# HandBrake/HandBrake

Hardware: AMD Instinct MI355X
Metric: filtered frames/sec, 1080p YUV420p NLMeans+decomb chain (higher is better)
Workload: dtype u8 (f32 NLMeans weights, 16-bit fixed-point scaler as zimg, sharpen mix = the reference's f64 expression, as one f32 multiply where init proves that equal); 1 GPU; BASELINE configs[3]: decomb(31, EEDI2 bob) -> nlmeans medium -> cropscale lanczos 1920x1080 -> 3840x2160 -> lapsharp, 1080i YUV420P 8-bit in, inputs resident in HBM; input=1920x1080, output=3840x2160, streams_per_gpu=1, content=interlaced, stream_frames=48, stage_streams=2, parallelism=1 GPU(s) x 1 independent stream(s), device=AMD Radeon Graphics (gfx950:sramecc+:xnack-, 256 CUs)

## Files before the change

handbrake_amd/csrc/eedi2.hip:

```cpp
#include "eedi2_common.h"
#include "eedi2_vote.h"
#include "eedi2_dirmap_vote.h"
#include "eedi2_dense.h"
#include "eedi2_engine.h"
#include "eedi2_mask_cells.h"
#include "eedi2_corner.h"

#include <atomic>
#include <algorithm>

namespace {

constexpr int PEAK = 255, NEUTRAL = 128;
constexpr int EEDI_MAX_FIELDS = EEDI_MAX_BATCH;
constexpr size_t GUARD = 32768;

__constant__ uint8_t c_limlut[33] = { 6, 6, 7, 7, 8, 8, 9, 9, 9, 10, 10, 11, 11, 12, 12, 12, 12, 12, 12, 12,
                                      12, 12, 12, 12, 12, 12, 12, 12, 12, 12, 12, 255, 255 };

constexpr int LIM_N = 33, LIM_PAD = 40;
__device__ __forceinline__ void lim_fill(uint8_t *tab, int tid)
{
    if (tid < LIM_N) tab[tid] = c_limlut[tid];
}
// ... 708 lines not shown
        {
            if (k == 1 && tid >= 64) break;
            const int i = tid + k * CD_W;
    #pragma unroll
            for (int m = 0; m < NM; m++)
            {
                const uint64_t w = __ballot(s_band[NS + m][i] == PEAK);
                if (lane == 0) s_bits[m][i >> 6] = w;
            }
        }
        __syncthreads();
    }
#ifdef HBHIP_DEV_STATS
    if (tid == 0) { CD_STAT(0, 1); CD_STAT(1, count != 0); CD_STAT(2, count); CD_STAT(7, dense); }
#endif
    if (R >= 4 && dense)
    {
        constexpr int RD = R >= 4 ? R : 1;
        const int lx = tid, px = x0 + lx, b = lx + CD_HALO - 1;
        const int startu = max(-px + 1, -maxdt), stopu = min(width - 2 - px, maxdt);
        uint64_t range = 0;
        if (stopu >= startu)
        {
            const int nb = stopu - startu + 1;
            range = (nb >= 64 ? ~0ull : ((1ull << nb) - 1ull)) << (startu + maxdt);
        }
        uint64_t win[RD + 2];
#pragma unroll
        for (int m = 0; m < RD + 2; m++) win[m] = calc_dir_window(s_bits[m], b - maxdt, lenmask);
        uint32_t up[RD], dn[RD], act = 0, inactive = 0;
#pragma unroll
        for (int j = 0; j < RD; j++)
        {
            const uint8_t *mr = &s_band[NS + j + 1][CD_HALO + lx];
            const bool a = px >= 1 && px < width - 1 && mr[0] == PEAK && (mr[-1] == PEAK || mr[1] == PEAK);
            const uint64_t pass = a ? range & win[j] & (__brevll(win[j + 2]) >> (64 - len)) : 0ull;
            const uint64_t npass = ~pass;
            up[j] = (uint32_t)(npass >> maxdt);
            dn[j] = __brev((uint32_t)npass << (31 - maxdt));
            act |= (uint32_t)a << j;
            inactive |= (up[j] | dn[j]) & ((2u << maxdt) - 1u);
        }
        if (__any(act != 0))
        {
            const uint32_t *tr = &s_tri[0][b];
            if (__all(inactive == 0))
                calc_dir_dense_vote<RD, false, RD, 0>(tr, maxdt, up, dn, act, nt13, nt19, &s_out[0][lx]);
            else
            {
                constexpr int RH = RD >= 8 ? RD / 2 : RD;
                calc_dir_dense_vote<RH, true, RD, 0>(tr, maxdt, up, dn, act, nt13, nt19, &s_out[0][lx]);
                if constexpr (RH < RD) calc_dir_dense_vote<RD - RH, true, RD, RH>(tr, maxdt, up, dn, act, nt13, nt19, &s_out[0][lx]);
            }
#ifdef HBHIP_DEV_STATS
            if (lane == 0) { CD_STAT(8, 1); CD_STAT(9, __all(inactive == 0)); }
#endif
        }
        __syncthreads();
    }
    else if (count)
    {
        for (int p = tid; p < count; p += CD_W)
        {
            const uint32_t id = s_list[p];
            const int j = (int)(id >> 8), lx = (int)(id & 255u), y = y0 + j, px = x0 + lx, b = lx + CD_HALO - 1;
            const int startu = max(-px + 1, -maxdt), stopu = min(width - 2 - px, maxdt);
            uint64_t pass = 0;
            if (stopu >= startu)
            {
                const int nb = stopu - startu + 1;
                pass = (nb >= 64 ? ~0ull : ((1ull << nb) - 1ull)) << (startu + maxdt);
                if (y != 1)          pass &= calc_dir_window(s_bits[j], b - maxdt, lenmask);
                if (y != height - 2) pass &= __brevll(calc_dir_window(s_bits[j + 2], b - maxdt, lenmask)) >> (64 - len);
            }
#ifdef HBHIP_DEV_STATS
            {
                int n = __popcll(pass), mx = n, sm = n, ln = 1;
                for (int o = 32; o; o >>= 1) { mx = max(mx, __shfl_xor(mx, o)); sm += __shfl_xor(sm, o); ln += __shfl_xor(ln, o); }
                const uint64_t act = __ballot(1);
                if (lane == __ffsll((unsigned long long)act) - 1) { CD_STAT(3, 1); CD_STAT(4, sm); CD_STAT(5, mx); CD_STAT(6, ln); }
            }
#endif
            const uint32_t *tr = &s_tri[j][b];
            int out;
            if (len <= 32)
                out = edge ? calc_dir_search<true, uint32_t>(tr, (uint32_t)pass, maxdt, y == 1, y == height - 2, nt13, nt19)
                           : calc_dir_search<false, uint32_t>(tr, (uint32_t)pass, maxdt, false, false, nt13, nt19);
            else
                out = edge ? calc_dir_search<true, uint64_t>(tr, pass, maxdt, y == 1, y == height - 2, nt13, nt19)
                           : calc_dir_search<false, uint64_t>(tr, pass, maxdt, false, false, nt13, nt19);
            s_out[j][lx] = (uint8_t)out;
        }
        __syncthreads();
    }
#pragma unroll
    for (int jr = 0; jr < R; jr += CD_W / 64)
    {
        const int j = jr + (tid >> 6), y = y0 + j, xb = x0 + 4 * lane;
        if (j < R && y < height && xb < pitch)
            *reinterpret_cast<uint32_t *>(Q.c + (size_t)y * pitch + xb) = pad_bytes(reinterpret_cast<const uint32_t *>(&s_out[j][0])[lane], xb, width, padv);
    }
}


__device__ __forceinline__ int dir_map_px(int u0, int u1, int u2, int c0, int c1, int c2, int n0, int n1, int n2,
                                          bool up_ok, bool dn_ok, int expand, const uint8_t *limlut)
{
    const bool h0 = up_ok && u0 != PEAK, h1 = up_ok && u1 != PEAK, h2 = up_ok && u2 != PEAK;
    const bool h3 = c0 != PEAK, h4 = !expand && c1 != PEAK, h5 = c2 != PEAK;
    const bool h6 = dn_ok && n0 != PEAK, h7 = dn_ok && n1 != PEAK, h8 = dn_ok && n2 != PEAK;
    const int u = h0 + h1 + h2 + h3 + h4 + h5 + h6 + h7 + h8;
    if (u < (expand ? 5 : 4)) return expand ? c1 : PEAK;
    int v0 = h0 ? u0 : ABSENT, v1 = h1 ? u1 : ABSENT, v2 = h2 ? u2 : ABSENT;
    int v3 = h3 ? c0 : ABSENT, v4 = h4 ? c1 : ABSENT, v5 = h5 ? c2 : ABSENT;
    int v6 = h6 ? n0 : ABSENT, v7 = h7 ? n1 : ABSENT, v8 = h8 ? n2 : ABSENT;
    int s0 = v0, s1 = v1, s2 = v2, s3 = v3, s4 = v4, s5 = v5, s6 = v6, s7 = v7, s8 = v8;
    const int mid = mid9(s0, s1, s2, s3, s4, s5, s6, s7, s8, u);
    const int lim = limlut[iabs(mid - NEUTRAL) >> 2];
    int sum = 0, count = 0;
    vote1(v0, mid, lim, sum, count); vote1(v1, mid, lim, sum, count); vote1(v2, mid, lim, sum, count);
    vote1(v3, mid, lim, sum, count); vote1(v4, mid, lim, sum, count); vote1(v5, mid, lim, sum, count);
    vote1(v6, mid, lim, sum, count); vote1(v7, mid, lim, sum, count); vote1(v8, mid, lim, sum, count);
    const int val = dmv_vote_avg(sum + mid, count + 1);
    if (expand) return count >= 5 ? (val & 0xff) : c1;
    if (count < 4 || (count < 5 && c1 == PEAK)) return PEAK;
    return val & 0xff;
}

__device__ __forceinline__ uint32_t ff_bytes(uint32_t v)
{
    return (((v & 0x7f7f7f7fu) + 0x01010101u) & v) & 0x80808080u;
}

constexpr uint32_t PK_ABSENT_HI = 0x7f00u;
__device__ __forceinline__ u16x2 limlut2(u16x2 i)
{
    const u16x2 g = pk_lt(pk1(7), i);
    const u16x2 l = __builtin_elementwise_min((u16x2)(((i - g) >> 1) + pk1(6)), pk1(12));
    const u16x2 big = pk_lt(pk1(30), i) * pk1(255);
    return __builtin_elementwise_max(l, big);
}
#define PK_BYTES(hi, lo, a, b) __builtin_amdgcn_perm((hi), (lo), 0x0c000c00u | ((uint32_t)(b) << 16) | (uint32_t)(a))

template <int PAIRS>
__device__ __forceinline__ uint32_t dir_map_quad(const Win12 &wu, const Win12 &wc, const Win12 &wd)
{
    return ::dir_map_quad<PAIRS>(wu.w0, wu.w1, wu.w2, wc.w0, wc.w1, wc.w2, wd.w0, wd.w1, wd.w2);
}

__global__ __launch_bounds__(256) void k_dir_map4(P3 P)
{
    FIELD_PLANE(P);
    const int x = 4 * (blockIdx.x * blockDim.x + threadIdx.x);
    const int y = blockIdx.y * blockDim.y + threadIdx.y;
    const int pitch = P.pitch[pl], width = P.width[pl], height = P.height[pl];
    if (x >= width || y >= height) return;
    uint8_t *o = Q.c + (size_t)y * pitch + x;
    if (maskless)
    {
        const int out[4] = { PEAK, PEAK, PEAK, PEAK };
        st4(o, out, x, width);
        return;
    }
    const uint8_t *dc = Q.b + (size_t)y * pitch + x;
    const uint32_t own = *reinterpret_cast<const uint32_t *>(dc);
    uint32_t res = own;
    if (y >= 1 && y < height - 1)
    {
        const uint32_t m0 = *reinterpret_cast<const uint32_t *>(Q.a + (size_t)y * pitch + x);
        const uint32_t work = (ff_bytes(m0) >> 7) & bytes_in(x, 1, width - 1);
        if (work)
        {
            asm volatile("" ::: "memory");
            const Win12 wc = ldwin(dc), wu = ldwin(dc - (ptrdiff_t)pitch), wd = ldwin(dc + (ptrdiff_t)pitch);
            const uint32_t votes = dir_map_quad<3>(wu, wc, wd);
            const uint32_t sel = (work << 8) - work;
            res = (res & ~sel) | (votes & sel);
        }
    }
    int out[4] = { (int)(res & 0xff), (int)((res >> 8) & 0xff), (int)((res >> 16) & 0xff), (int)(res >> 24) };
    st4(o, out, x, width);
}

__device__ __forceinline__ uint32_t live3(const Win12 &w, uint32_t &centre)
{
    const uint32_t n0 = (~ff_bytes(w.w0) >> 7) & 0x01010101u, n1 = (~ff_bytes(w.w1) >> 7) & 0x01010101u, n2 = (~ff_bytes(w.w2) >> 7) & 0x01010101u;
    centre = n1;
    return __builtin_amdgcn_alignbyte(n1, n0, 3) + n1 + __builtin_amdgcn_alignbyte(n2, n1, 1);
}

#ifndef DC_THREAD_ROWS
#define DC_THREAD_ROWS 4
#endif
constexpr int DC_R = DC_THREAD_ROWS, DC_ROWS = 4 * DC_R;
__global__ __launch_bounds__(256) void k_dir_map_c(P3 P)
{
    __shared__ __attribute__((aligned(16))) uint8_t s_out[DC_ROWS][256];
    __shared__ uint16_t s_list[DC_ROWS * 256];
    __shared__ int s_count;
    __shared__ uint8_t s_lim[LIM_PAD];
    FIELD_PLANE(P);
    const int rb = blockIdx.y * DC_ROWS;
    const int bx0 = 4 * (blockIdx.x * 64), x = bx0 + 4 * threadIdx.x;
    const int pitch = P.pitch[pl], width = P.width[pl], height = P.height[pl];
    if (bx0 >= width || rb >= height) return;
    if (maskless)
    {
        if (x < width)
        {
            const int out[4] = { PEAK, PEAK, PEAK, PEAK };
#pragma unroll
            for (int h = 0; h < DC_R; h++)
            {
                const int y = rb + (int)threadIdx.y + 4 * h;
                if (y < height) st4(Q.c + (size_t)y * pitch + x, out, x, width);
            }
        }
        return;
    }
    const int tid = threadIdx.y * 64 + threadIdx.x;
    if (tid == 0) s_count = 0;
    lim_fill(s_lim, tid);
    __syncthreads();
    uint32_t own[DC_R], m0[DC_R], cand[DC_R];
#pragma unroll
    for (int h = 0; h < DC_R; h++)
    {
        const int y = rb + (int)threadIdx.y + 4 * h;
        own[h] = 0; m0[h] = 0;
        if (x < width && y < height)
        {
            own[h] = *reinterpret_cast<const uint32_t *>(Q.b + (size_t)y * pitch + x);
            if (y >= 1 && y < height - 1)
                m0[h] = *reinterpret_cast<const uint32_t *>(Q.a + (size_t)y * pitch + x);
        }
    }
    Win12 wc[DC_R], wu[DC_R], wd[DC_R];
#pragma unroll
    for (int h = 0; h < DC_R; h++)
    {
        const int y = rb + (int)threadIdx.y + 4 * h;
        cand[h] = (ff_bytes(m0[h]) >> 7) & bytes_in(x, 1, width - 1) & (ff_bytes(own[h]) >> 7);
        wc[h] = wu[h] = wd[h] = Win12{ 0u, 0u, 0u };
        if (cand[h])
        {
            const uint8_t *dc = Q.b + (size_t)y * pitch + x;
            wc[h] = ldwin(dc); wu[h] = ldwin(dc - (ptrdiff_t)pitch); wd[h] = ldwin(dc + (ptrdiff_t)pitch);
        }
    }
#pragma unroll
    for (int h = 0; h < DC_R; h++)
    {
        const int lr = (int)threadIdx.y + 4 * h, y = rb + lr;
        if (x < width && y < height)
        {
            if (cand[h])
            {
                uint32_t nc, nu, nd;
                const uint32_t s3c = live3(wc[h], nc), s3u = live3(wu[h], nu), s3d = live3(wd[h], nd);
                const uint32_t u = s3c - nc + s3u + s3d;
                const uint32_t enough = ((u + (uint32_t)(0x80 - 5) * 0x01010101u) >> 7) & 0x01010101u;
                const uint32_t sortpx = cand[h] & enough;
                if (sortpx)
                {
                    int at = atomicAdd(&s_count, __popc(sortpx));
#pragma unroll
                    for (int k = 0; k < 4; k++)
                        if ((sortpx >> (8 * k)) & 1u) s_list[at++] = (uint16_t)((lr << 8) | (4 * threadIdx.x + k));
                }
                (void)nu; (void)nd;
            }
            *reinterpret_cast<uint32_t *>(&s_out[lr][4 * threadIdx.x]) = own[h];
        }
    }
    __syncthreads();
    const int count = s_count;
    for (int i = tid; i < count; i += 256)
    {
        const int e = s_list[i], ly = e >> 8, lx = e & 255;
        const uint8_t *c = Q.b + (size_t)(rb + ly) * pitch + bx0 + lx;
        const uint8_t *up = c - (ptrdiff_t)pitch, *dn = c + (ptrdiff_t)pitch;
        s_out[ly][lx] = (uint8_t)dir_map_px(up[-1], up[0], up[1], c[-1], c[0], c[1], dn[-1], dn[0], dn[1], true, true, 1, s_lim);
    }
    __syncthreads();
#pragma unroll
    for (int h = 0; h < DC_R; h++)
    {
        const int lr = (int)threadIdx.y + 4 * h, y = rb + lr;
        if (x < width && y < height)
        {
            const uint32_t v = *reinterpret_cast<const uint32_t *>(&s_out[lr][4 * threadIdx.x]);
            uint8_t *o = Q.c + (size_t)y * pitch + x;
            if (x + 3 < width) *reinterpret_cast<uint32_t *>(o) = v;
            else for (int k = 0; k < 4 && x + k < width; k++) o[k] = (uint8_t)(v >> (8 * k));
        }
    }
}

#ifndef FE_ROWS
#define FE_ROWS 14
#endif
constexpr int FE_R = FE_ROWS, FE_LW = 68;

__device__ __forceinline__ void fe_expand_row(const uint32_t (*s_f)[FE_LW], int lr, int tx, uint32_t cand, bool up_ok, bool dn_ok,
                                              uint8_t (*s_out)[256], uint16_t *s_list, int *s_count)
{
    const uint32_t own = s_f[lr + 1][tx + 1];
    cand &= ff_bytes(own) >> 7;
    if (cand)
    {
        const Win12 none = { 0xffffffffu, 0xffffffffu, 0xffffffffu };
        const Win12 wc = { s_f[lr + 1][tx], own, s_f[lr + 1][tx + 2] };
        const Win12 wu = up_ok ? Win12{ s_f[lr][tx], s_f[lr][tx + 1], s_f[lr][tx + 2] } : none;
        const Win12 wd = dn_ok ? Win12{ s_f[lr + 2][tx], s_f[lr + 2][tx + 1], s_f[lr + 2][tx + 2] } : none;
        uint32_t nc, nu, nd;
        const uint32_t s3c = live3(wc, nc), s3u = live3(wu, nu), s3d = live3(wd, nd);
        const uint32_t u = s3c - nc + s3u + s3d;
        const uint32_t enough = ((u + (uint32_t)(0x80 - 5) * 0x01010101u) >> 7) & 0x01010101u;
        const uint32_t sortpx = cand & enough;
        if (sortpx)
        {
            int at = atomicAdd(s_count, __popc(sortpx));
#pragma unroll
            for (int k = 0; k < 4; k++)
                if ((sortpx >> (8 * k)) & 1u) s_list[at++] = (uint16_t)((lr << 8) | (4 * tx + k));
        }
        (void)nu; (void)nd;
    }
    *reinterpret_cast<uint32_t *>(&s_out[lr][4 * tx]) = own;
}

template <int STEP, bool POST>
__global__ __launch_bounds__(256) void k_dir_map_fe(P3 P, uint32_t padv)
{
    __shared__ uint32_t s_f[FE_R + 2][FE_LW];
    __shared__ __attribute__((aligned(16))) uint8_t s_out[FE_R][256];
    __shared__ uint16_t s_list[FE_R * 256];
    __shared__ int s_count;
    __shared__ uint8_t s_lim[LIM_PAD];
    FIELD_PLANE(P);
    const int y0 = STEP == 1 ? 1 : 2 - tff, par = STEP == 1 ? 0 : (y0 & 1);
    const int rb = blockIdx.y * FE_R;
    const int bx0 = 256 * blockIdx.x, x = bx0 + 4 * threadIdx.x;
    const int pitch = P.pitch[pl], width = P.width[pl], height = P.height[pl];
    if (bx0 >= pitch || STEP * rb >= height) return;
    auto row_ok = [&](int y) { return STEP == 1 ? (y >= 1 && y < height - 1) : (y >= y0 && y < height - 1); };
    if (maskless)
    {
        if (x < pitch)
            for (int lr = threadIdx.y; lr < FE_R; lr += 4)
#pragma unroll
                for (int i = 0; i < STEP; i++)
                    if (STEP * (rb + lr) + i < height)
                    {
                        const size_t at = (size_t)(STEP * (rb + lr) + i) * pitch + x;
                        *reinterpret_cast<uint32_t *>(Q.c + at) = pad_bytes(0xffffffffu, x, width, padv);
                        if (POST && x < width) { const int out[4] = { PEAK, PEAK, PEAK, PEAK }; st4(Q.d + at, out, x, width); }
                    }
        return;
    }
    const int tid = threadIdx.y * 64 + threadIdx.x;
    if (tid == 0) s_count = 0;
    lim_fill(s_lim, tid);
    constexpr int NCOPY = STEP == 1 ? 1 : (FE_R + 3) / 4;
    uint32_t vcopy[NCOPY];
    if (STEP != 1)
#pragma unroll
        for (int h = 0; h < NCOPY; h++)
        {
            const int lr = threadIdx.y + 4 * h, yc = 2 * (rb + lr) + 1 - par;
            vcopy[h] = (lr < FE_R && yc < height && x < width) ? *reinterpret_cast<const uint32_t *>(Q.b + (size_t)yc * pitch + x) : 0u;
        }
    auto filtered = [&](int r, int xx, auto side) -> uint32_t {
        constexpr int SIDE = decltype(side)::value;
        const int y = STEP * r + par;
        if (r < 0 || y >= height || xx < 0 || xx >= width) return 0u;
        const uint8_t *dc = Q.b + (size_t)y * pitch + xx;
        const uint32_t own = *reinterpret_cast<const uint32_t *>(dc);
        if (!row_ok(y)) return own;
        const uint8_t *mk = Q.a + (size_t)y * pitch + xx;
        const uint32_t m0 = *reinterpret_cast<const uint32_t *>(STEP == 1 ? mk : mk - (ptrdiff_t)pitch);
        const uint32_t m1 = STEP == 1 ? 0u : *reinterpret_cast<const uint32_t *>(mk + pitch);
        uint32_t work = ((ff_bytes(m0) | ff_bytes(m1)) >> 7) & bytes_in(xx, 1, width - 1);
        if (SIDE < 0) work &= 0xff000000u;
        if (SIDE > 0) work &= 0x000000ffu;
        uint32_t res = own;
        if (work)
        {
            asm volatile("" ::: "memory");
            const bool up_ok = STEP == 1 || y > 1, dn_ok = STEP == 1 || y < height - 2;
            const Win12 none = { 0xffffffffu, 0xffffffffu, 0xffffffffu };
            const Win12 wc = ldwin(dc), wu = up_ok ? ldwin(dc - (ptrdiff_t)STEP * pitch) : none, wd = dn_ok ? ldwin(dc + (ptrdiff_t)STEP * pitch) : none;
            const uint32_t votes = dir_map_quad<(SIDE < 0 ? 2 : SIDE > 0 ? 1 : 3)>(wu, wc, wd);
            const uint32_t sel = (work << 8) - work;
            res = (res & ~sel) | (votes & sel);
        }
        return res;
    };
    for (int lr = threadIdx.y; lr < FE_R + 2; lr += 4) s_f[lr][threadIdx.x + 1] = filtered(rb - 1 + lr, x, std::integral_constant<int, 0>());
    static_assert(FE_R + 2 <= 64, "a lane per ring row");
    if (threadIdx.y == 0 && (int)threadIdx.x < FE_R + 2) s_f[threadIdx.x][0] = filtered(rb - 1 + (int)threadIdx.x, bx0 - 4, std::integral_constant<int, -1>());
    if (threadIdx.y == 1 && (int)threadIdx.x < FE_R + 2) s_f[threadIdx.x][65] = filtered(rb - 1 + (int)threadIdx.x, bx0 + 256, std::integral_constant<int, 1>());
    __syncthreads();
    for (int lr = threadIdx.y; lr < FE_R; lr += 4)
    {
        const int y = STEP * (rb + lr) + par;
        if (x >= width || y >= height) continue;
        uint32_t cand = 0;
        if (row_ok(y))
        {
            const uint8_t *mk = Q.a + (size_t)y * pitch + x;
            const uint32_t m0 = *reinterpret_cast<const uint32_t *>(STEP == 1 ? mk : mk - (ptrdiff_t)pitch);
            const uint32_t m1 = STEP == 1 ? 0u : *reinterpret_cast<const uint32_t *>(mk + pitch);
            cand = ((ff_bytes(m0) | ff_bytes(m1)) >> 7) & bytes_in(x, 1, width - 1);
        }
        fe_expand_row(s_f, lr, threadIdx.x, cand, STEP == 1 || y > 1, STEP == 1 || y < height - 2, s_out, s_list, &s_count);
    }
    __syncthreads();
    const int count = s_count;
    for (int i = tid; i < count; i += 256)
    {
        const int e = s_list[i], ly = e >> 8, lx = e & 255;
        const int y = STEP * (rb + ly) + par;
        const uint8_t *c = reinterpret_cast<const uint8_t *>(&s_f[ly + 1][1]) + lx;
        const uint8_t *up = c - 4 * FE_LW, *dn = c + 4 * FE_LW;
        s_out[ly][lx] = (uint8_t)dir_map_px(up[-1], up[0], up[1], c[-1], c[0], c[1], dn[-1], dn[0], dn[1],
                                            STEP == 1 || y > 1, STEP == 1 || y < height - 2, 1, s_lim);
    }
    __syncthreads();
#pragma unroll
    for (int h = 0; h < (FE_R + 3) / 4; h++)
    {
        const int lr = threadIdx.y + 4 * h, y = STEP * (rb + lr) + par;
        if (lr >= FE_R || x >= pitch) continue;
        auto put_d = [&](int yy, uint32_t v) {
            if (x >= width) return;
            uint8_t *o = Q.d + (size_t)yy * pitch + x;
            if (x + 3 < width) *reinterpret_cast<uint32_t *>(o) = v;
            else for (int k = 0; k < 4 && x + k < width; k++) o[k] = (uint8_t)(v >> (8 * k));
        };
        if (y < height)
        {
            const uint32_t v = x < width ? *reinterpret_cast<const uint32_t *>(&s_out[lr][4 * threadIdx.x]) : 0u;
            *reinterpret_cast<uint32_t *>(Q.c + (size_t)y * pitch + x) = pad_bytes(v, x, width, padv);
            if (POST) put_d(y, s_f[lr + 1][threadIdx.x + 1]);
            if (POST && x < width && row_ok(y))
            {
                const size_t at = (size_t)y * pitch + x;
                const uint32_t om4 = *reinterpret_cast<const uint32_t *>(Q.b + at);
                uint8_t *d = Q.f + at;
                const uint32_t up4 = *reinterpret_cast<const uint32_t *>(d - pitch), dn4 = *reinterpret_cast<const uint32_t *>(d + pitch);
                const uint32_t cur4 = *reinterpret_cast<const uint32_t *>(d);
                int out[4];
                bool any = false;
#pragma unroll
                for (int k = 0; k < 4; k++)
                {
                    const int nm = (v >> (8 * k)) & 0xffu, om = (om4 >> (8 * k)) & 0xffu;
                    const int lim = s_lim[iabs(nm - NEUTRAL) >> 2];
                    const bool fix = iabs(nm - om) > lim && om != PEAK && om != NEUTRAL;
                    out[k] = fix ? (int)((((up4 >> (8 * k)) & 0xffu) + ((dn4 >> (8 * k)) & 0xffu) + 1) >> 1) : (int)((cur4 >> (8 * k)) & 0xffu);
                    any |= fix;
                }
                if (any) st4(d, out, x, width);
            }
        }
        if (STEP != 1)
        {
            const int yc = 2 * (rb + lr) + 1 - par;
            if (yc < height)
            {
                *reinterpret_cast<uint32_t *>(Q.c + (size_t)yc * pitch + x) = pad_bytes(vcopy[h < NCOPY ? h : 0], x, width, padv);
                if (POST) put_d(yc, vcopy[h < NCOPY ? h : 0]);
            }
        }
    }
}


constexpr int FM_W = 256, FM_R = 4, FM_HALO = 8, FM_LW = FM_W + 2 * FM_HALO;

__device__ __forceinline__ int fm_step(uint32_t s, uint32_t c, uint32_t ref, int lim)
{
    const int off_s = lim - (int)__builtin_amdgcn_sad_u16(s, ref, 0u), off_c = lim - (int)__builtin_amdgcn_sad_u16(c, ref, 0u);
    return (off_s & (int)(s - 255u)) | (off_c & (int)(c - 255u)) | (509 - (int)c - (int)s);
}

__global__ __launch_bounds__(256) void k_filter_map(P3 P)
{
    __shared__ __attribute__((aligned(16))) uint8_t s_d[FM_R + 2][FM_LW];
    FIELD_PLANE(P);
    const int pitch = P.pitch[pl], width = P.width[pl], height = P.height[pl];
    const int bx0 = blockIdx.x * FM_W, by0 = blockIdx.y * FM_R;
    if (bx0 >= width || by0 >= height) return;
    const int tid = threadIdx.y * 64 + threadIdx.x;
    const int x = bx0 + 4 * threadIdx.x, y = by0 + threadIdx.y;
    if (maskless)
    {
        if (x < width && y < height)
        {
            uint8_t *o = Q.c + (size_t)y * pitch + x;
            if (x + 3 < width) *reinterpret_cast<uint32_t *>(o) = 0xffffffffu;
            else for (int k = 0; k < 4 && x + k < width; k++) o[k] = (uint8_t)PEAK;
        }
        return;
    }
    const bool inside = x < width && y < height;
    uint32_t m4 = 0, own = 0;
    if (inside)
    {
        own = *reinterpret_cast<const uint32_t *>(Q.b + (size_t)y * pitch + x);
        if (y >= 1 && y < height - 1) m4 = *reinterpret_cast<const uint32_t *>(Q.a + (size_t)y * pitch + x);
    }
    uint32_t cand = ((ff_bytes(m4) & ~ff_bytes(own)) >> 7) & bytes_in(x, 1, width - 1);
    if (!__syncthreads_or(cand != 0u))
    {
        if (inside)
        {
            uint8_t *o = Q.c + (size_t)y * pitch + x;
            if (x + 3 < width) *reinterpret_cast<uint32_t *>(o) = own;
            else for (int k = 0; k < 4 && x + k < width; k++) o[k] = (uint8_t)(own >> (8 * k));
        }
        return;
    }
    {
        static_assert((FM_R + 2) * (FM_LW / 4) <= 2 * 256, "two staged dwords per thread");
        uint32_t v[2] = { 0u, 0u };
#pragma unroll
        for (int k = 0; k < 2; k++)
        {
            const int i = tid + 256 * k, r = i / (FM_LW / 4), c4 = i - r * (FM_LW / 4);
            const int yy = by0 - 1 + r, col = bx0 - FM_HALO + 4 * c4;
            if (i < (FM_R + 2) * (FM_LW / 4) && yy >= 0 && yy < height && col >= 0 && col < pitch)
                v[k] = *reinterpret_cast<const uint32_t *>(Q.b + (size_t)yy * pitch + col);
        }
#pragma unroll
        for (int k = 0; k < 2; k++)
            if (tid + 256 * k < (FM_R + 2) * (FM_LW / 4)) reinterpret_cast<uint32_t *>(&s_d[0][0])[tid + 256 * k] = v[k];
    }
    __syncthreads();
    if (!inside) return;
    const uint8_t *rc = &s_d[threadIdx.y + 1][FM_HALO + 4 * threadIdx.x];
    uint32_t out4 = own;
#pragma unroll 1
    for (int k = 0; k < 4; k++)
    {
        if (!((cand >> (8 * k)) & 1u)) continue;
        const int xx = x + k;
        const uint8_t *dc = rc + k, *dp = dc - FM_LW, *dn = dc + FM_LW;
        const uint32_t ref = dc[0];
        int dir = ((int)ref - NEUTRAL) >> 2;
        const int lim = max(iabs(dir) * 2, 12 << 2);
        dir >>= 2;
        const int neg = min(dir, 0), pos = max(dir, 0);
        const int tf = max(-xx, neg), tt = min(width - xx - 1, pos), bf = max(-xx, -pos), bt = min(width - xx - 1, -neg);
        const int n = max(tt - tf, bt - bf);
        int any_t = 0, any_b = 0;
        for (int i = 0; i <= n; i++)
        {
            const int jt = min(tf + i, tt), jb = min(bf + i, bt);
            any_t |= fm_step(dp[jt], dc[jt], ref, lim);
            any_b |= fm_step(dn[jb], dc[jb], ref, lim);
        }
        if ((any_t & any_b) < 0) out4 |= 0xffu << (8 * k);
    }
    uint8_t *o = Q.c + (size_t)y * pitch + x;
    if (x + 3 < width) *reinterpret_cast<uint32_t *>(o) = out4;
    else for (int k = 0; k < 4 && x + k < width; k++) o[k] = (uint8_t)(out4 >> (8 * k));
}

template <int K>
__device__ __forceinline__ uint32_t mark_pair(const Win12 &wa, const Win12 &wb)
{
    u16x2 v[6];
    {
        const Win12 *rows[2] = { &wa, &wb };
#pragma unroll
        for (int r = 0; r < 2; r++)
        {
            const uint32_t w0 = rows[r]->w0, w1 = rows[r]->w1, w2 = rows[r]->w2;
            if (K == 0)
            {
                v[3 * r + 0] = pk(PK_BYTES(w1, w0, 3, 4));
                v[3 * r + 1] = pk(PK_BYTES(w1, w0, 4, 5));
                v[3 * r + 2] = pk(PK_BYTES(w1, w0, 5, 6));
            }
            else
            {
                v[3 * r + 0] = pk(PK_BYTES(w1, w0, 5, 6));
                v[3 * r + 1] = pk(PK_BYTES(w1, w0, 6, 7));
                v[3 * r + 2] = pk(PK_BYTES(w2, w1, 3, 4));
            }
        }
    }
    const u16x2 one = pk1(1), zero = pk1(0);
    u16x2 a[6], raw[6];
    uint32_t absent = 0;
#pragma unroll
    for (int i = 0; i < 6; i++)
    {
        raw[i] = v[i];
        a[i] = (u16x2)((v[i] + one) >> 8);
        absent += un(a[i]);
        v[i] = v[i] + a[i] * pk1(PK_ABSENT_HI);
    }
    u16x2 s0 = v[0], s1 = v[1], s2 = v[2], s3 = v[3], s4 = v[4], s5 = v[5];
    cswap2(s0, s5); cswap2(s1, s3); cswap2(s2, s4);
    cswap2(s1, s2); cswap2(s3, s4);
    cswap2(s0, s3); cswap2(s2, s5);
    cswap2(s0, s1); cswap2(s2, s3); cswap2(s4, s5);
    cswap2(s1, s2); cswap2(s3, s4);
    const u16x2 ab = pk(absent);
    const uint32_t m4 = un(zero - pk_lt(one, ab));
    const uint32_t m3 = un(zero - pk_lt(pk1(2), ab));
    const uint32_t m5 = un(zero - pk_lt(zero, ab));
    const uint32_t modd = un(zero - (ab & one));
#define PK_SEL(m, x, y) (((m) & (x)) | (~(m) & (y)))
    const uint32_t lo = PK_SEL(m4, un(s1), un(s2));
    const uint32_t hi = PK_SEL(m3, un(s1), PK_SEL(m5, un(s2), un(s3)));
    const u16x2 mid = pk(PK_SEL(modd, hi, un((u16x2)((pk(lo) + pk(hi) + one) >> 1))));
#undef PK_SEL
    const i16x2 t = __builtin_bit_cast(i16x2, (u16x2)(mid - pk1(NEUTRAL)));
    const u16x2 lim1 = limlut2(__builtin_bit_cast(u16x2, __builtin_elementwise_max(t, (i16x2)(-t))) >> 2) + one;
    auto close = [&](int i, int j, int k) -> u16x2 {
        const u16x2 d = __builtin_elementwise_max(raw[i], raw[j]) - __builtin_elementwise_min(raw[i], raw[j]);
        return pk_lt(d, lim1) | a[i] | a[k];
    };
    const u16x2 u = close(0, 3, 3) + close(1, 4, 4) + close(2, 3, 5);
    u16x2 sum = zero, cnt = zero;
#pragma unroll
    for (int i = 0; i < 6; i++)
    {
        const u16x2 d = __builtin_elementwise_max(v[i], mid) - __builtin_elementwise_min(v[i], mid);
        const u16x2 in = pk_lt(d, lim1);
        cnt += in;
        sum += in * v[i];
    }
    const uint32_t sm = un((u16x2)(sum + mid)), ct = un(cnt), uu = un(u);
    uint32_t out = 0;
#pragma unroll
    for (int h = 0; h < 2; h++)
    {
        const int n = 6 - (int)((absent >> (16 * h)) & 0xffffu);
        const int count = (int)((ct >> (16 * h)) & 0xffffu);
        int res = PEAK;
        if (n >= 3 && (int)((uu >> (16 * h)) & 0xffffu) >= 2 && !(count < n - 2 || count < 2))
            res = vote_avg((int)((sm >> (16 * h)) & 0xffffu), count + 1) & 0xff;
        out |= (uint32_t)res << (16 * h);
    }
    return out;
}


__global__ __launch_bounds__(256) void k_mark_2x4(P3 P, uint32_t padv)
{
    FIELD_PLANE(P);
    const int x = 4 * (blockIdx.x * blockDim.x + threadIdx.x);
    const int r = blockIdx.y * blockDim.y + threadIdx.y;
    const int pitch = P.pitch[pl], width = P.width[pl], height = P.height[pl];
    const int y0 = 2 - tff;
    if (x >= pitch || 2 * r >= height) return;
    const bool two = 2 * r + 1 < height;
    const int y = 2 * r + (y0 & 1), yc = 2 * r + 1 - (y0 & 1);
    const bool rebuilt = y < height && !maskless && y >= y0 && y < height - 1;
    const size_t hs = (size_t)r * pitch + x, fs = (size_t)(2 * r) * pitch + x;
    const uint32_t vg = *reinterpret_cast<const uint32_t *>(Q.g + hs), vb = *reinterpret_cast<const uint32_t *>(Q.b + hs),
                   va = *reinterpret_cast<const uint32_t *>(Q.a + hs);
    uint32_t k0w = 0, k1w = 0;
    if (rebuilt)
    {
        const int ra = (y - 1) >> 1, rb = (y + 1) >> 1;
        k0w = ra == r ? va : *reinterpret_cast<const uint32_t *>(Q.a + (ptrdiff_t)ra * pitch + x);
        k1w = rb == r ? va : *reinterpret_cast<const uint32_t *>(Q.a + (ptrdiff_t)rb * pitch + x);
    }
    const bool vote = rebuilt && ((ff_bytes(k0w) | ff_bytes(k1w)) & bytes_in(x, 1, width - 1)) != 0u;
    Win12 wa = { 0u, 0u, 0u }, wbn = { 0u, 0u, 0u };
    if (vote)
    {
        wa = ldwin(Q.b + (ptrdiff_t)((y - 1) >> 1) * pitch + x);
        wbn = ldwin(Q.b + (ptrdiff_t)((y + 1) >> 1) * pitch + x);
    }
    {
        *reinterpret_cast<uint32_t *>(Q.d + fs) = vg;
        *reinterpret_cast<uint32_t *>(Q.e + fs) = vb;
        *reinterpret_cast<uint32_t *>(Q.f + fs) = va;
        if (two)
        {
            *reinterpret_cast<uint32_t *>(Q.d + fs + pitch) = vg;
            *reinterpret_cast<uint32_t *>(Q.e + fs + pitch) = vb;
            *reinterpret_cast<uint32_t *>(Q.f + fs + pitch) = va;
        }
    }
    if (yc < height) *reinterpret_cast<uint32_t *>(Q.c + (size_t)yc * pitch + x) = pad_bytes(0xffffffffu, x, width, padv);
    if (y >= height) return;
    uint32_t *o = reinterpret_cast<uint32_t *>(Q.c + (size_t)y * pitch + x);
    uint32_t packed = 0xffffffffu;
    if (!vote)
    {
        *o = pad_bytes(packed, x, width, padv);
        return;
    }
    {
        const uint32_t work = ((ff_bytes(k0w) | ff_bytes(k1w)) >> 7) & bytes_in(x, 1, width - 1);
        asm volatile("" ::: "memory");
        const uint32_t p01 = mark_pair<0>(wa, wbn), p23 = mark_pair<2>(wa, wbn);
        const uint32_t votes = __builtin_amdgcn_perm(p23, p01, 0x06040200u);
        const uint32_t sel = work * 255u;
        packed = (packed & ~sel) | (votes & sel);
    }
    *o = pad_bytes(packed, x, width, padv);
}

#ifndef FG_WIDTH
#define FG_WIDTH 1024
#endif
constexpr int FG_W = FG_WIDTH, FG_T = FG_W / 4, FG_HALO = 64, FG_LW = FG_W + 2 * FG_HALO;


#ifndef FG_ROWS
#define FG_ROWS 4
#endif
constexpr int FG_R = FG_ROWS, FG_ND = FG_R + 2, FG_NM = FG_R + 3, FG_WORDS = FG_LW / 64 + 1;
__global__ __launch_bounds__(FG_T) void k_fill_gaps_b(P3 P)
{
    __shared__ __attribute__((aligned(16))) uint8_t s_d[FG_ND][FG_LW];
    __shared__ __attribute__((aligned(16))) uint8_t s_m[FG_NM][FG_LW];
    __shared__ __attribute__((aligned(16))) uint8_t s_out[FG_R][FG_W];
    __shared__ uint16_t s_list[FG_R * FG_W];
    __shared__ int s_count;
    __shared__ uint64_t s_stop[FG_R][FG_WORDS], s_np[FG_R][FG_WORDS], s_bt[FG_R][FG_WORDS], s_bb[FG_R][FG_WORDS];
    FIELD_PLANE(P);
    const int y0 = 2 - tff;
    const int pitch = P.pitch[pl], width = P.width[pl], height = P.height[pl];
    const int x0 = blockIdx.x * FG_W, tid = threadIdx.x;
    const int ya = (int)blockIdx.y * 2 * FG_R;
    if (ya >= height || x0 >= width) return;
    const int yb = ya + (y0 & 1);
    const int x = x0 + 4 * tid;
    if (maskless)
    {
        if (x + 3 < width)
        {
#pragma unroll
            for (int i = 0; i < 2 * FG_R && ya + i < height; i++)
                *reinterpret_cast<uint32_t *>(Q.c + (size_t)(ya + i) * pitch + x) = 0xffffffffu;
        }
        else if (x < width)
            for (int i = 0; i < 2 * FG_R && ya + i < height; i++)
                for (int k = 0; k < 4 && x + k < width; k++) Q.c[(size_t)(ya + i) * pitch + x + k] = (uint8_t)PEAK;
        return;
    }
    auto rebuilt = [&](int y) { return y >= y0 && y < height - 1; };
    uint32_t vcopy[2 * FG_R] = {};
    if (x < width)
    {
#pragma unroll
        for (int i = 0; i < 2 * FG_R; i++)
        {
            const int y = ya + i;
            if (y < height && !((((y - y0) & 1) == 0) && rebuilt(y)))
                vcopy[i] = *reinterpret_cast<const uint32_t *>(Q.b + (size_t)y * pitch + x);
        }
    }
    if (tid == 0) s_count = 0;
    const int lo = x0 - FG_HALO;
    const int ndw = (min(FG_W, hbhip_align_up_dev(width - x0, 4)) + 2 * FG_HALO) / 4;
    {
        const bool h0 = tid < ndw, h1 = tid + FG_T < ndw;
        const int i0 = min(tid, ndw - 1), i1 = min(tid + FG_T, ndw - 1);
        uint32_t vd[FG_ND][2], vm[FG_NM][2];
#pragma unroll
        for (int r = 0; r < FG_ND; r++)
        {
            const uint32_t *row = reinterpret_cast<const uint32_t *>(Q.b + (size_t)min(max(yb - 2 + 2 * r, 0), height - 1) * pitch + lo);
            vd[r][0] = row[i0]; vd[r][1] = row[i1];
        }
#pragma unroll
        for (int r = 0; r < FG_NM; r++)
        {
            const uint32_t *row = reinterpret_cast<const uint32_t *>(Q.a + (size_t)min(max(yb - 3 + 2 * r, 0), height - 1) * pitch + lo);
            vm[r][0] = row[i0]; vm[r][1] = row[i1];
        }
        if (h0)
        {
#pragma unroll
            for (int r = 0; r < FG_ND; r++) reinterpret_cast<uint32_t *>(s_d[r])[tid] = vd[r][0];
#pragma unroll
            for (int r = 0; r < FG_NM; r++) reinterpret_cast<uint32_t *>(s_m[r])[tid] = vm[r][0];
        }
        if (h1)
        {
#pragma unroll
            for (int r = 0; r < FG_ND; r++) reinterpret_cast<uint32_t *>(s_d[r])[tid + FG_T] = vd[r][1];
#pragma unroll
            for (int r = 0; r < FG_NM; r++) reinterpret_cast<uint32_t *>(s_m[r])[tid + FG_T] = vm[r][1];
        }
    }
    __syncthreads();
    const unsigned staged = 4u * (unsigned)ndw;
#pragma unroll
    for (int r = 0; r < FG_R; r++)
    {
        const int y = yb + 2 * r;
        if (y < height && rebuilt(y))
        {
            uint32_t gap = 0u;
            if (x < width)
            {
                const int c = 4 * tid + FG_HALO;
                const uint32_t cw = *reinterpret_cast<const uint32_t *>(&s_d[r + 1][c]);
                const uint32_t mcw = *reinterpret_cast<const uint32_t *>(&s_m[r + 1][c]), mnw = *reinterpret_cast<const uint32_t *>(&s_m[r + 2][c]);
                *reinterpret_cast<uint32_t *>(&s_out[r][4 * tid]) = cw;
                gap = ((ff_bytes(cw) & (ff_bytes(mcw) | ff_bytes(mnw))) >> 7) & bytes_in(x, 1, width - 1);
            }
            int at = wave_list_slots(&s_count, (unsigned)__popc(gap));
#pragma unroll
            for (int k = 0; k < 4; k++)
                if ((gap >> (8 * k)) & 1u) s_list[at++] = (uint16_t)((r << 12) | (4 * tid + k));
        }
    }
    __syncthreads();
    const int count = s_count;
#ifdef HBHIP_DEV_STATS
    if (tid == 0) CD_STAT(12, 1);
#endif
    if (count)
    {
        for (int k = 0; k < (FG_LW + FG_T - 1) / FG_T; k++)
        {
            const unsigned col = tid + FG_T * k, cc = min(col, staged - 1u);
            uint64_t nd[FG_ND], pm[FG_NM];
    #pragma unroll
            for (int r = 0; r < FG_ND; r++) nd[r] = __ballot(s_d[r][cc] != PEAK);
    #pragma unroll
            for (int r = 0; r < FG_NM; r++) pm[r] = __ballot(s_m[r][cc] == PEAK);
            if ((tid & 63) == 0 && (col >> 6) < (unsigned)FG_WORDS)
            {
    #pragma unroll
                for (int r = 0; r < FG_R; r++)
                {
                    const uint64_t mc = pm[r + 1], mn = pm[r + 2];
                    s_np[r][col >> 6] = nd[r + 1];
                    s_stop[r][col >> 6] = nd[r + 1] | ~(mc | mn);
                    s_bt[r][col >> 6] = ~(nd[r] & (pm[r] | mc));
                    s_bb[r][col >> 6] = ~(nd[r + 2] & (mn | pm[r + 3]));
                }
            }
        }
        __syncthreads();
    }
    for (int i = tid; i < count; i += FG_T)
    {
        const int e = s_list[i], r = e >> 12, lx = e & 0xfff, px = x0 + lx, y = yb + 2 * r;
        const uint8_t *DC = s_d[r + 1], *DP = s_d[r], *DN = s_d[r + 2];
        const uint8_t *MC = s_m[r + 1], *MN = s_m[r + 2], *MP = s_m[r], *MNN = s_m[r + 3];
        const uint8_t *gd = Q.b + (size_t)y * pitch, *gma = Q.a + (ptrdiff_t)(y - 1) * pitch;
        auto rd = [&](const uint8_t *srow, const uint8_t *grow, int col) -> int {
            const unsigned k = (unsigned)(col - lo);
            return k < staged ? (int)srow[k] : (int)grow[col];
        };
        int u = px - 1, back = 500, forward = -500;
        int v = px + 1;
        int tc = 1, bc = 1, mint = 500, maxt = -20, minb = 500, maxb = -20;
        const int c = px - lo;
        const int first = max(1 - lo, 0), last = min((int)staged, width - lo);
        int ul = -1, vl = -1;
        for (int wi = (c - 1) >> 6; wi >= (first >> 6) && c - 1 >= first; wi--)
        {
            uint64_t w = s_stop[r][wi];
            if (wi == ((c - 1) >> 6) && ((c - 1) & 63) != 63) w &= (2ull << ((c - 1) & 63)) - 1ull;
            if (wi == (first >> 6)) w &= ~0ull << (first & 63);
            if (w) { ul = 64 * wi + 63 - __clzll((long long)w); break; }
        }
        for (int wi = (c + 1) >> 6; wi <= ((last - 1) >> 6) && c + 1 < last; wi++)
        {
            uint64_t w = s_stop[r][wi];
            if (wi == ((c + 1) >> 6)) w &= ~0ull << ((c + 1) & 63);
            if (wi == ((last - 1) >> 6) && ((last - 1) & 63) != 63) w &= (2ull << ((last - 1) & 63)) - 1ull;
            if (w) { vl = 64 * wi + __ffsll((long long)w) - 1; break; }
        }
        const bool fast = (ul >= 0 || lo <= 1) && (vl >= 0 || lo + (int)staged > width);
        if (fast)
        {
            if (ul >= 0) { u = lo + ul; if ((s_np[r][ul >> 6] >> (ul & 63)) & 1ull) back = DC[ul]; }
            else u = 0;
            if (vl >= 0) { v = lo + vl; if ((s_np[r][vl >> 6] >> (vl & 63)) & 1ull) forward = DC[vl]; }
            else v = width;
            const int a0 = u - lo, a1 = v - lo;
            auto any_in = [&](const uint64_t *bits) {
                for (int wi = a0 >> 6; wi <= (a1 >> 6); wi++)
                {
                    uint64_t w = bits[wi];
                    if (wi == (a0 >> 6)) w &= ~0ull << (a0 & 63);
                    if (wi == (a1 >> 6) && (a1 & 63) != 63) w &= (2ull << (a1 & 63)) - 1ull;
                    if (w) return true;
                }
                return false;
            };
            if (y <= 2 || any_in(s_bt[r])) { tc = 0; mint = maxt = 20; }
            else for (int j = a0; j <= a1; j++) { const int t = DP[j]; mint = min(mint, t); maxt = max(maxt, t); }
            if (y >= height - 3 || any_in(s_bb[r])) { bc = 0; minb = maxb = 20; }
            else for (int j = a0; j <= a1; j++) { const int t = DN[j]; minb = min(minb, t); maxb = max(maxb, t); }
        }
        else
        {
            const uint8_t *gmn = gma + 2 * (ptrdiff_t)pitch;
            while (u)
            {
                const int d = rd(DC, gd, u);
                if (d != PEAK) { back = d; break; }
                if (rd(MC, gma, u) != PEAK && rd(MN, gmn, u) != PEAK) break;
                u--;
            }
            while (v < width)
            {
                const int d = rd(DC, gd, v);
                if (d != PEAK) { forward = d; break; }
                if (rd(MC, gma, v) != PEAK && rd(MN, gmn, v) != PEAK) break;
                v++;
            }
            const uint8_t *gdp = gd - 2 * (ptrdiff_t)pitch, *gdn = gd + 2 * (ptrdiff_t)pitch;
            const uint8_t *gmp = gma - 2 * (ptrdiff_t)pitch, *gmnn = gmn + 2 * (ptrdiff_t)pitch;
            for (int j = u; j <= v; j++)
            {
                if (tc)
                {
                    int t;
                    if (y <= 2 || (t = rd(DP, gdp, j)) == PEAK || (rd(MP, gmp, j) != PEAK && rd(MC, gma, j) != PEAK)) { tc = 0; mint = maxt = 20; }
                    else { mint = min(mint, t); maxt = max(maxt, t); }
                }
                if (bc)
                {
                    int t;
                    if (y >= height - 3 || (t = rd(DN, gdn, j)) == PEAK || (rd(MN, gmn, j) != PEAK && rd(MNN, gmnn, j) != PEAK)) { bc = 0; minb = maxb = 20; }
                    else { minb = min(minb, t); maxb = max(maxb, t); }
                }
            }
        }
#ifdef HBHIP_DEV_STATS
        CD_STAT(13, 1); CD_STAT(14, v - u); CD_STAT(15, fast); CD_STAT(16, tc + bc); CD_STAT(17, (tc + bc) * (v - u + 1));
#endif
        if (maxt == -20) maxt = mint = 20;
        if (maxb == -20) maxb = minb = 20;
        const int far = max(iabs(forward - NEUTRAL), iabs(back - NEUTRAL));
        const int thresh = max(max(far >> 2, 8), max(iabs(mint - maxt), iabs(minb - maxb)));
        const int flim = min(far >> 2, 6);
        if (iabs(forward - back) <= thresh && (v - u - 1 <= flim || tc || bc))
        {
            const double stepd = (double)(forward - back) / (double)(v - u);
            const int j = px - u - 1;
            s_out[r][lx] = (uint8_t)((back + (int)(j * stepd + 0.5)) & 0xff);
        }
    }
    __syncthreads();
    auto out_word = [&](int i) -> uint32_t {
        const int y = ya + i;
        const bool work = (((y - y0) & 1) == 0) && rebuilt(y);
        return work ? *reinterpret_cast<const uint32_t *>(&s_out[(i - (y0 & 1)) >> 1][4 * tid]) : vcopy[i];
    };
    if (x + 3 < width)
    {
#pragma unroll
// ... 960 lines not shown
```

Measured before the change: 10050 output frames/s.

## Remap lanes onto live columns in partial edge tiles for EEDI2 dir-map and mark

Adds a LaneMap that, for the right-edge block where only part of the 256-byte tile lies inside the pitch, reassigns wave/lane work units so every lane covers a live column and row instead of idling past the edge. The fill and expand loops of k_dir_map_fe, its right halo column, and k_mark_2x4 use this mapping, so partial blocks do less divergent, wasted work. It adds index arithmetic and more complex control flow, and the rotating wave-to-unit mapping in k_mark_2x4 relies on the 4-row blocking staying correct.

```diff
diff --git a/handbrake_amd/csrc/eedi2.hip b/handbrake_amd/csrc/eedi2.hip
--- a/handbrake_amd/csrc/eedi2.hip
+++ b/handbrake_amd/csrc/eedi2.hip
@@ -1034,6 +1034,21 @@
 #endif
 constexpr int FE_R = FE_ROWS, FE_LW = 68;
 
+struct LaneMap
+{
+    int live, ncg, shift, wave, lane;
+    __device__ __forceinline__ LaneMap(int bx0, int pitch)
+        : live(min(4, (pitch - bx0 + 63) >> 6)), ncg(live == 3 ? 3 : 1),
+          shift(live == 4 ? 6 : live == 2 ? 5 : 4),
+          wave(__builtin_amdgcn_readfirstlane((int)threadIdx.y)), lane((int)threadIdx.x) {}
+    __device__ __forceinline__ void unit(int u, int &tx, int &row) const
+    {
+        const int step = ncg == 3 ? (u * 11) >> 5 : u, cg = u - step * ncg;
+        tx = (cg << shift) + (lane & ((1 << shift) - 1));
+        row = ((step << 6) + lane) >> shift;
+    }
+};
+
 __device__ __forceinline__ void fe_expand_row(const uint32_t (*s_f)[FE_LW], int lr, int tx, uint32_t cand, bool up_ok, bool dn_ok,
                                               uint8_t (*s_out)[256], uint16_t *s_list, int *s_count)
 {
@@ -1073,12 +1088,13 @@
     FIELD_PLANE(P);
     const int y0 = STEP == 1 ? 1 : 2 - tff, par = STEP == 1 ? 0 : (y0 & 1);
     const int rb = blockIdx.y * FE_R;
-    const int bx0 = 256 * blockIdx.x, x = bx0 + 4 * threadIdx.x;
+    const int bx0 = 256 * blockIdx.x;
     const int pitch = P.pitch[pl], width = P.width[pl], height = P.height[pl];
     if (bx0 >= pitch || STEP * rb >= height) return;
     auto row_ok = [&](int y) { return STEP == 1 ? (y >= 1 && y < height - 1) : (y >= y0 && y < height - 1); };
     if (maskless)
     {
+        const int x = bx0 + 4 * threadIdx.x;
         if (x < pitch)
             for (int lr = threadIdx.y; lr < FE_R; lr += 4)
 #pragma unroll
@@ -1092,6 +1108,8 @@
         return;
     }
     const int tid = threadIdx.y * 64 + threadIdx.x;
+    const int x = bx0 + 4 * threadIdx.x;
+    const LaneMap lm(bx0, pitch);
     if (tid == 0) s_count = 0;
     lim_fill(s_lim, tid);
     constexpr int NCOPY = STEP == 1 ? 1 : (FE_R + 3) / 4;
@@ -1129,25 +1147,45 @@
         }
         return res;
     };
-    for (int lr = threadIdx.y; lr < FE_R + 2; lr += 4) s_f[lr][threadIdx.x + 1] = filtered(rb - 1 + lr, x, std::integral_constant<int, 0>());
+    static_assert(FE_R + 2 <= 16, "4 live units");
+    if (lm.live == 4)
+        for (int lr = threadIdx.y; lr < FE_R + 2; lr += 4) s_f[lr][threadIdx.x + 1] = filtered(rb - 1 + lr, x, std::integral_constant<int, 0>());
+    else
+        for (int i = 0; i < lm.live; i++)
+        {
+            int tx, lr;
+            lm.unit(lm.wave + 4 * i, tx, lr);
+            if (lr < FE_R + 2) s_f[lr][tx + 1] = filtered(rb - 1 + lr, bx0 + 4 * tx, std::integral_constant<int, 0>());
+        }
     static_assert(FE_R + 2 <= 64, "a lane per ring row");
-    if (threadIdx.y == 0 && (int)threadIdx.x < FE_R + 2) s_f[threadIdx.x][0] = filtered(rb - 1 + (int)threadIdx.x, bx0 - 4, std::integral_constant<int, -1>());
-    if (threadIdx.y == 1 && (int)threadIdx.x < FE_R + 2) s_f[threadIdx.x][65] = filtered(rb - 1 + (int)threadIdx.x, bx0 + 256, std::integral_constant<int, 1>());
+    if ((int)threadIdx.x < FE_R + 2)
+    {
+        if (lm.wave == 0) s_f[threadIdx.x][0] = filtered(rb - 1 + (int)threadIdx.x, bx0 - 4, std::integral_constant<int, -1>());
+        if (lm.wave == 1) s_f[threadIdx.x][16 * lm.live + 1] = filtered(rb - 1 + (int)threadIdx.x, bx0 + 64 * lm.live, std::integral_constant<int, 1>());
+    }
     __syncthreads();
-    for (int lr = threadIdx.y; lr < FE_R; lr += 4)
-    {
-        const int y = STEP * (rb + lr) + par;
-        if (x >= width || y >= height) continue;
+    auto expand_at = [&](int tx, int lr) {
+        const int xe = bx0 + 4 * tx, y = STEP * (rb + lr) + par;
+        if (lr >= FE_R || xe >= width || y >= height) return;
         uint32_t cand = 0;
         if (row_ok(y))
         {
-            const uint8_t *mk = Q.a + (size_t)y * pitch + x;
+            const uint8_t *mk = Q.a + (size_t)y * pitch + xe;
             const uint32_t m0 = *reinterpret_cast<const uint32_t *>(STEP == 1 ? mk : mk - (ptrdiff_t)pitch);
             const uint32_t m1 = STEP == 1 ? 0u : *reinterpret_cast<const uint32_t *>(mk + pitch);
-            cand = ((ff_bytes(m0) | ff_bytes(m1)) >> 7) & bytes_in(x, 1, width - 1);
-        }
-        fe_expand_row(s_f, lr, threadIdx.x, cand, STEP == 1 || y > 1, STEP == 1 || y < height - 2, s_out, s_list, &s_count);
-    }
+            cand = ((ff_bytes(m0) | ff_bytes(m1)) >> 7) & bytes_in(xe, 1, width - 1);
+        }
+        fe_expand_row(s_f, lr, tx, cand, STEP == 1 || y > 1, STEP == 1 || y < height - 2, s_out, s_list, &s_count);
+    };
+    if (lm.live == 4)
+        for (int lr = threadIdx.y; lr < FE_R; lr += 4) expand_at(threadIdx.x, lr);
+    else
+        for (int i = 0; i < lm.live; i++)
+        {
+            int tx, lr;
+            lm.unit(lm.wave + 4 * i, tx, lr);
+            expand_at(tx, lr);
+        }
     __syncthreads();
     const int count = s_count;
     for (int i = tid; i < count; i += 256)
@@ -1387,9 +1425,18 @@
 __global__ __launch_bounds__(256) void k_mark_2x4(P3 P, uint32_t padv)
 {
     FIELD_PLANE(P);
-    const int x = 4 * (blockIdx.x * blockDim.x + threadIdx.x);
-    const int r = blockIdx.y * blockDim.y + threadIdx.y;
     const int pitch = P.pitch[pl], width = P.width[pl], height = P.height[pl];
+    if (256 * (int)blockIdx.x >= pitch) return;
+    int tx = threadIdx.x, ty = threadIdx.y;
+    if (!maskless)
+    {
+        const LaneMap lm(256 * (int)blockIdx.x, pitch);
+        const int u = (lm.wave - lm.live * (int)blockIdx.y) & 3;
+        if (u >= lm.live) return;
+        lm.unit(u, tx, ty);
+    }
+    const int x = 4 * (blockIdx.x * 64 + tx);
+    const int r = blockIdx.y * 4 + ty;
     const int y0 = 2 - tff;
     if (x >= pitch || 2 * r >= height) return;
     const bool two = 2 * r + 1 < height;
```

After: 10110 output frames/s (median of 6 runs). About the same (+0.6%).
